# matthiasverstraete/3d_recognizer

Hardware: AMD Instinct MI355X
Metric: training clouds/sec, N=40960 pts, bs=8, at 1/2/4/8 GPUs; mIoU parity (higher is better)
Workload: dtype f32 storage/accumulate, bf16x3 MFMA in the wide GEMMs

## Files before the change

### 3d_recognizer_amd/csrc/pool.hip

```cpp
#include <string.h>

#include "rl_common.h"
#include <stdlib.h>

namespace {

#ifdef RL_POOL_PLAIN_STORES
#define RL_ST1 rl_stx
#define RL_ST4 rl_stx4
#else
#define RL_ST1 rl_stx_nt
#define RL_ST4 rl_stx4_nt
#endif

typedef float f32x4 __attribute__((ext_vector_type(4)));
typedef __attribute__((ext_vector_type(4))) __bf16 bf16x4;
typedef __attribute__((ext_vector_type(8))) __bf16 bf16x8;
typedef __attribute__((ext_vector_type(4))) short s16x4;

typedef float f32x2 __attribute__((ext_vector_type(2)));
typedef __attribute__((ext_vector_type(2))) __bf16 bf16x2;
__device__ __forceinline__ void split2(const f32x2 x, unsigned& hi, unsigned& lo) {
    const unsigned hb = __builtin_bit_cast(unsigned, __builtin_convertvector(x, bf16x2));
    const f32x2 hf = {__uint_as_float(hb << 16), __uint_as_float(hb & 0xffff0000u)};
// ... 569 lines not shown
#pragma unroll
                    for (int r = 0; r < 4; ++r) accw[nb][kb][r] += red[((nb * DT + kb) * 4 + r) * 64 + lane];
        }
    }
    if (wave == 0) {
        float* out = p.slab + (long)blockIdx.x * p.slab_stride;
#pragma unroll
        for (int nb = 0; nb < DT; ++nb)
#pragma unroll
            for (int kb = 0; kb < DT; ++kb)
#pragma unroll
                for (int r = 0; r < 4; ++r) out[(long)(nb * 16 + lj * 4 + r) * D + kb * 16 + li] = accw[nb][kb][r];
    }
}

template <bool GB, bool XO = true>
__global__ __launch_bounds__(512) void pool128_bwd_kernel(const PoolParams p) {
    __shared__ __attribute__((aligned(16))) float lfm[LFold<8>::LDS_FLOATS];
    constexpr int NW = 8;
    constexpr int TERMS = 3;
    constexpr int DT = 8, D = 128, H = 64, XS = Tile<DT>::XS, XSB = Tile<DT>::XSB;
    __shared__ __attribute__((aligned(16))) __bf16 Wh[D * XSB];
    __shared__ __attribute__((aligned(16))) __bf16 Wl[D * XSB];
    __shared__ __attribute__((aligned(16))) float Tiles[NW][16 * XS];
    const int lane = threadIdx.x & 63, wave = __builtin_amdgcn_readfirstlane(threadIdx.x >> 6);
    const int li = lane & 15, lj = lane >> 4;
    for (int e = threadIdx.x; e < D * D; e += 64 * NW) {
        const int o = e / D, i = e - o * D;
        const float w = p.W[e];
        const __bf16 h = (__bf16)w;
        Wh[o * XSB + i] = h;
        if constexpr (TERMS == 3) Wl[o * XSB + i] = (__bf16)(w - (float)h);
    }
    LFold<DT> lf;
    lf.init(p, lj, lfm);
    __syncthreads();
    float* Xs = Tiles[wave];
    float* Ds = Tiles[wave];

    const PointSpan span = point_span<NW>(p, wave);
    const long pstep = span.step, Pend = span.end;
    long pt = span.first;
    int idx_cur = pt < Pend ? p.idx[pt * 16 + li] : 0;
    int idx_nxt = pt + pstep < Pend ? p.idx[(pt + pstep) * 16 + li] : 0;
    float4 raw[DT];
    Cursor cu;
    cu.start(pt, p.n);
    float gp[DT], gp_nxt[DT];
#pragma unroll
    for (int nb = 0; nb < DT; ++nb) gp[nb] = gp_nxt[nb] = 0.f;
    if (pt < Pend) {
        fetch_x<DT>(p, cu, li, lj, idx_cur, raw);
#pragma unroll
        for (int nb = 0; nb < DT; ++nb) gp[nb] = p.dP[pt * D + nb * 16 + li];
    }
    loads_landed();
    for (; pt < Pend; pt += pstep) {
        const Cursor cn = cu.next(pstep, p.n);
        float4 xa[DT];
        finish_x<DT>(p, li, lj, raw, lf, xa, Xs);
        const int idx_n2 = pt + 2 * pstep < Pend ? p.idx[(pt + 2 * pstep) * 16 + li] : 0;
        const Cursor cf = pt + pstep < Pend ? cn : cu;
        fetch_x<DT>(p, cf, li, lj, pt + pstep < Pend ? idx_nxt : idx_cur, raw);
#pragma unroll
        for (int nb = 0; nb < DT; ++nb) gp_nxt[nb] = p.dP[cf.pt * D + nb * 16 + li];
        loads_issued();
        cu = cn;
        idx_cur = idx_nxt; idx_nxt = idx_n2;
        if constexpr (XO)
#pragma unroll
            for (int c = 0; c < DT; ++c) rl_stx4<GB>(p.X_out, (pt * 16 + li) * D + 16 * c + 4 * lj, xa[c]);
        f32x4 a[DT];
#pragma unroll
        for (int nb = 0; nb < DT; ++nb) a[nb] = (f32x4){0.f, 0.f, 0.f, 0.f};
        tile_gemm_bf<DT>(xa, Wh, Wl, li, lj, a);
// ... 54 lines not shown
        __builtin_amdgcn_wave_barrier();
        const long orow = (pt * 16 + li) * H;
        float4 gold[DT / 2];
        if (p.gu_accumulate) {
#pragma unroll
            for (int c = 0; c < DT / 2; ++c) gold[c] = *reinterpret_cast<const float4*>(p.GU + orow + 16 * c + 4 * lj);
        }
#pragma unroll
        for (int c = DT / 2; c < DT; ++c)
            rl_stx4<GB>(p.DG, orow + 16 * c + 4 * lj - H, *reinterpret_cast<const float4*>(Ds + li * XS + 16 * c + 4 * lj));
#pragma unroll
        for (int c = 0; c < DT / 2; ++c) {
            f32x4 v = *reinterpret_cast<const f32x4*>(Ds + li * XS + 16 * c + 4 * lj);
            if (p.gu_accumulate) v += v4(gold[c]);
            *reinterpret_cast<float4*>(p.GU + orow + 16 * c + 4 * lj) = f4(v);
        }
#pragma unroll
        for (int nb = 0; nb < DT; ++nb) gp[nb] = gp_nxt[nb];
        __builtin_amdgcn_wave_barrier();
    }
}

struct RpeBwdParams {
    PoolParams pp;
    const float* G;
    double* stats;
    const float* coef;
    float* slab;
    float* GU1;
    int g_bf16;
};

__device__ __forceinline__ float li_sum(float v) {
    v += __shfl_xor(v, 1, 64); v += __shfl_xor(v, 2, 64); v += __shfl_xor(v, 4, 64); v += __shfl_xor(v, 8, 64);
// ... 1419 lines not shown
#pragma unroll
        for (int j = 0; j < 16; ++j) t += red[j][ex];
        dW[e] = t;
    }
}

enum PoolEntry { PE_FWD, PE_BWD, PE_STATS, PE_BN_REDUCE, PE_WGRAD };

struct PoolFacts {
    PoolEntry entry;
    int d, stage;
    int terms;
    bool rows_bf16, gu_accumulate, fwd_stats2;
    long points;
    bool skip_x;
};

typedef void (*PoolFn)();
struct PoolPlan {
    PoolFn fn;
    int grid, threads;
    int xcd_chunk;
    int dw_count;
    const char* name;
    const char* refusal;
};

constexpr int pool_wavefronts(bool virtual_bwd, int d) { return d == 128 || (virtual_bwd && d == 64) ? 8 : 4; }

template <template <int, int> class Pick, class... A>
PoolFn by_width(int d, int terms, A... a) {
    if (terms == 0) return d == 16 ? Pick<1, 0>::fn(a...) : d == 32 ? Pick<2, 0>::fn(a...) : Pick<4, 0>::fn(a...);
    return d == 16 ? Pick<1, 3>::fn(a...) : d == 32 ? Pick<2, 3>::fn(a...) : Pick<4, 3>::fn(a...);
}
template <int DT, int T> struct PoolFwd { static PoolFn fn() { return (PoolFn)pool_fwd_kernel<DT, T>; } };
template <int DT, int T> struct PoolBwd {
    static PoolFn fn(bool gb) {
        if constexpr (T == 3) if (gb) return (PoolFn)pool_bwd_kernel<DT, 3, false, 4, true>;
        return (PoolFn)pool_bwd_kernel<DT, T>;
// ... 30 lines not shown
    pl.threads = 64 * nw;
    const long per = 4 * nw;
    const long cap = rpe ? RL_MAX_SLOTS : nw == 8 ? 256 : (fwd && d <= 16) ? 1280 : (fwd && d == 64) ? 768 : 1024;
    const long g = (f.points + per - 1) / per;
    pl.grid = (int)(g < 1 ? 1 : g < cap ? g : cap);
    if (((fwd && virt) || f.entry == PE_STATS) && pl.grid >= 8 && pl.grid % 8 == 0 && f.points < (1l << 30))
        pl.xcd_chunk = (int)((f.points + 7) / 8);

    if (!(d == 16 || d == 32 || d == 64 || (d == 128 && !virt && !rpe && f.terms != 0))) {
        pl.refusal = "d must be 16, 32 or 64, or 128 with a stored U outside the fp32 arithmetic mode";
        return pl;
    }
    const bool gb = f.rows_bf16 && !fwd && f.entry != PE_STATS;
    if (gb && f.terms != 3 && d != 128) { pl.refusal = "bf16 gradient rows need the bf16x3 arithmetic mode"; return pl; }
    if (f.skip_x && gb) { pl.refusal = "bf16 gradient rows need X_out (the in-place X of the weight gradient is fp32 only)"; return pl; }
    switch (f.entry) {
    case PE_FWD:
        pl.name = virt ? "vpool_fwd_kernel" : d == 16 ? "pool_fwd_kernel<1>" : d == 32 ? "pool_fwd_kernel<2>" : d == 64 ? "pool_fwd_kernel<4>" : "pool_fwd_kernel<8>";
        pl.fn = virt ? by_width<VPoolFwd>(d, f.terms, s2, f.fwd_stats2)
              : d == 128 ? (PoolFn)pool_fwd_kernel<8, 3, pool_wavefronts(false, 128)> : by_width<PoolFwd>(d, f.terms);
        break;
    case PE_BWD:
        pl.name = virt ? "vpool_bwd_kernel" : d == 16 ? "pool_bwd_kernel<1>" : d == 32 ? "pool_bwd_kernel<2>" : d == 64 ? "pool_bwd_kernel<4>" : "pool128_bwd_kernel";
        pl.fn = virt ? by_width<VPoolBwd>(d, f.terms, s2, gb, f.gu_accumulate)
              : d == 128 ? (gb ? (PoolFn)pool128_bwd_kernel<true> : f.skip_x ? (PoolFn)pool128_bwd_kernel<false, false> : (PoolFn)pool128_bwd_kernel<false>)
              : by_width<PoolBwd>(d, f.terms, gb);
        pl.dw_count = d == 128 ? 0 : d * d;
        break;
    case PE_STATS:
        pl.name = "vrpe_stats_kernel";
        pl.fn = by_width<RpeStats>(d, f.terms, s2);
        break;
    case PE_BN_REDUCE:
    case PE_WGRAD:
        pl.name = f.entry == PE_WGRAD ? "vrpe_wgrad_kernel" : "vrpe_bn_reduce_kernel";
        pl.fn = by_width<RpeBwd>(d, f.terms, s2, gb, f.entry == PE_WGRAD);
        break;
    }
    return pl;
}

template <class... Args>
int launch_pool(const PoolPlan& pl, const char* who, void* stream, const float* slab, float* dW, Args... args) {
    hipStream_t st = (hipStream_t)stream;
    void (*fn)(Args...) = (void (*)(Args...))pl.fn;
    hipLaunchKernelGGL(fn, dim3(pl.grid), dim3(pl.threads), 0, st, args...);
    rl_note_kernel(pl.name);
    RL_LAUNCH_CHECK(who);
    if (dW) {
        hipLaunchKernelGGL(pool_dw_reduce_kernel, dim3(rl_cdiv(pl.dw_count, 16)), dim3(256), 0, st, slab, pl.grid, pl.dw_count, dW);
        RL_LAUNCH_CHECK(who);
    }
    return RL_OK;
// ... 45 lines not shown
    if (rc) return rc;
    RL_REQUIRE(d->G && d->W && (p->src > 0 || d->U) && d->g_bstride >= d->n, RL_ERR_ARGS, "%s: null G / W / U, or g_bstride < n", who);
    RL_REQUIRE((p->src > 0 || ((uintptr_t)d->U & 15) == 0) && ((uintptr_t)d->G & 15) == 0, RL_ERR_ARGS, "%s: U/G must be 16-byte aligned", who);
    RL_REQUIRE((d->u_scale == nullptr) == (d->u_shift == nullptr) && (d->g_scale == nullptr) == (d->g_shift == nullptr),
               RL_ERR_ARGS, "%s: scale/shift must come together", who);
    p->U = d->U; p->ulazy.scale = d->u_scale; p->ulazy.shift = d->u_shift; p->ulazy.act = d->u_act; p->ulazy.slope = d->u_slope;
    p->G = d->G; p->g_bstride = d->g_bstride;
    p->glazy.scale = d->g_scale; p->glazy.shift = d->g_shift; p->glazy.act = d->g_act; p->glazy.slope = d->g_slope;
    p->W = d->W;
    p->Pout = d->Pout; p->dP = d->dP; p->GU = d->GU; p->gu_accumulate = d->gu_accumulate; p->DG = d->DG; p->slab = d->slab;
    p->slab_stride = (long)d->d * d->d + (d->dW ? 0 : d->d);
    if (backward) p->piv1 = p->piv2 = nullptr;
    p->fstats2 = backward ? nullptr : d->bn_fwd_stats2;
    RL_REQUIRE(!p->fstats2 || (p->src == 1 && d->W2 && d->b2), RL_ERR_ARGS, "%s: bn_fwd_stats2 needs virtual stage 1 and W2 / b2", who);
    p->bstats = backward ? d->bn_bwd_stats : nullptr;
    RL_REQUIRE(!p->bstats || p->src > 0, RL_ERR_ARGS, "%s: bn_bwd_stats needs a virtual rpe stage", who);
    RL_REQUIRE(backward ? (d->dP && d->GU && d->DG) : d->Pout != nullptr, RL_ERR_ARGS, "%s: null output / gradient buffers", who);
    return RL_OK;
}

int plan_grid(PoolEntry entry, int64_t points, int d, int stage) { return plan_pool({entry, d, stage, rl_wide_terms(), false, false, false, points}).grid; }

}

extern "C" int rl_pool_supported(int d, int nbr_k) { return nbr_k == 16 && !plan_pool({PE_FWD, d, 0, rl_wide_terms(), false, false, false, 1}).refusal; }

extern "C" int64_t rl_pool_slab_floats(int64_t points, int d) {
    const int stored = plan_grid(PE_BWD, points, d, 0), virt = plan_grid(PE_BWD, points, d, 1);
    return (int64_t)(stored > virt ? stored : virt) * (d * d + d);
}
extern "C" int rl_pool_bwd_slots(int64_t points, int d) { return plan_grid(PE_BWD, points, d, 1); }
// ... 3 lines not shown
extern "C" int64_t rl_rpe_wgrad_slab_floats(int64_t points, int d, int stage) {
    const int h = d / 2;
    return (int64_t)plan_grid(PE_WGRAD, points, d, stage) * ((int64_t)h * (stage == 1 ? 10 : h) + h);
}

extern "C" int rl_pool_fwd(const rl_pool_desc* d, void* stream) {
    PoolParams p;
    int rc = fill(&p, d, "rl_pool_fwd", false);
    if (rc) return rc;
    const PoolPlan pl = plan_pool({PE_FWD, p.d, p.src, rl_wide_terms(), false, false, p.fstats2 != nullptr, p.P});
    RL_REQUIRE(!pl.refusal, RL_ERR_UNSUPPORTED, "rl_pool_fwd: %s (d %d, u_source %d)", pl.refusal, p.d, p.src);
    p.xcd_chunk = pl.xcd_chunk;
    return launch_pool(pl, "rl_pool_fwd", stream, nullptr, nullptr, p);
}

extern "C" int rl_pool_bwd(const rl_pool_desc* d, void* stream) {
    PoolParams p;
    int rc = fill(&p, d, "rl_pool_bwd", true);
    if (rc) return rc;
    const bool skip_x = p.d == 128 && d->x_optional != 0 && d->X_out == nullptr;
    const PoolPlan pl = plan_pool({PE_BWD, p.d, p.src, rl_wide_terms(), d->rows_bf16 != 0, p.gu_accumulate != 0, false, p.P, skip_x});
    RL_REQUIRE(!pl.refusal, RL_ERR_UNSUPPORTED, "rl_pool_bwd: %s (d %d, u_source %d)", pl.refusal, p.d, p.src);
    if (p.d == 128) {
        RL_REQUIRE((d->X_out || skip_x) && d->dS_out, RL_ERR_ARGS, "rl_pool_bwd: d = 128 needs X_out and dS_out");
        RL_REQUIRE((((uintptr_t)d->X_out | (uintptr_t)d->dS_out) & 15) == 0, RL_ERR_ARGS, "rl_pool_bwd: X_out / dS_out must be 16-byte aligned");
        p.X_out = d->X_out; p.dS_out = d->dS_out;
        return launch_pool(pl, "rl_pool_bwd", stream, nullptr, nullptr, p);
    }
    RL_REQUIRE(d->slab, RL_ERR_ARGS, "rl_pool_bwd: null gradient buffers");
    RL_REQUIRE(d->slab_floats >= (int64_t)pl.grid * p.slab_stride, RL_ERR_ARGS, "rl_pool_bwd: slab too small");
    return launch_pool(pl, "rl_pool_bwd", stream, p.slab, d->dW, p);
}

static int g_pool128_x_in_place = 1;
extern "C" int rl_set_pool128_x(const char* mode) {
    const bool in_place = mode && !strcmp(mode, "in_place"), stored = mode && !strcmp(mode, "stored");
    RL_REQUIRE(in_place || stored, RL_ERR_ARGS, "rl_set_pool128_x: mode must be \"in_place\" or \"stored\"");
    g_pool128_x_in_place = in_place ? 1 : 0;
    return RL_OK;
}
extern "C" const char* rl_get_pool128_x(void) { return g_pool128_x_in_place ? "in_place" : "stored"; }

extern "C" int rl_rpe_stats(const rl_pool_desc* d, double* stats, void* stream) {
    PoolParams p;
    int rc = fill_branch(&p, d, "rl_rpe_stats", BN_BELOW);
    if (rc) return rc;
    RL_REQUIRE(p.src > 0 && stats, RL_ERR_ARGS, "rl_rpe_stats: needs u_source 1 or 2 and a stats buffer");
// ... 41 lines not shown
```

### 3d_recognizer_amd/randlanet/_engine.py

```python
from dataclasses import dataclass, field
from typing import ClassVar, Dict, List, Optional

import torch

from . import _hip as H
from . import _ops as ops
from ._ops import Lazy, Rpe

BN_EPS = 1e-6
BN_MOMENTUM = 0.99
BN_PIVOT = True
BAND_SORT_MIN_POINTS = 4096
POOL_X_IN_PLACE_MIN_ROWS = 2048
DECODER_CAT_IN_PLACE_MIN_ROWS = 8192


@dataclass(slots=True, eq=False)
class _Record:
    kind: ClassVar[str] = ""
    level: int = field(default=-1, init=False)


@dataclass(slots=True, eq=False)
class LinearRec(_Record):
    kind: ClassVar[str] = "linear"
    a: object
    out: Lazy
    wname: str
    bname: Optional[str]
# ... 17 lines not shown
    d: int


@dataclass(slots=True, eq=False)
class PoolFusedRec(_Record):
    kind: ClassVar[str] = "pool_fused"
    name: str
    u: object
    g: Lazy
    csr: object
    idx: torch.Tensor
    pooled: Lazy
    n: int
    d: int
    stage: int


@dataclass(slots=True, eq=False)
class AddActRec(_Record):
    kind: ClassVar[str] = "add_act"
    m2: Lazy
    sc: Lazy
    O: Lazy


@dataclass(slots=True, eq=False)
class InterpConcatRec(_Record):
    kind: ClassVar[str] = "interp_concat"
    prev: Lazy
    skip: Lazy
# ... 207 lines not shown
        for Y, (wname, bname, bn, n_out, act, slope, ks, ns, stats), last in zip(res, metas, (first_is_last_consumer, 0)):
            out = Lazy(Y, a.B, a.n, a.n, n_out)
            self._bn(ctx, out, stats, bn, act, slope, folded_bias=self.P[bname],
                     nslots=H.row_blocks(out.rows, 128) if stats is not None else None)
            ctx.record(LinearRec(a, out, wname, bname, ks, ns, True, last))
            outs.append(out)
        return outs[0], outs[1]

    def _mlp(self, ctx, a, name: str, n_out: int, act: int = H.ACT_NONE, slope: float = 0.0, *, transposed=False,
             bn=True, a_grad=True, last_consumer_of_input: int = 0) -> Lazy:
        return self._linear(ctx, a, f"{name}.conv.weight", f"{name}.conv.bias", n_out, transposed=transposed,
                            bn=f"{name}.batch_norm" if bn else None, act=act, slope=slope, a_grad=a_grad,
                            last_consumer_of_input=last_consumer_of_input)

    def _pool(self, ctx, name: str, u, g: Lazy, idx: torch.Tensor, csr, n: int, d: int, n_out: int, stage: int = 0,
              next_stats: bool = False) -> Lazy:
        B, K, h = u.B, self.K, d // 2
        rows = B * n * K
        Ws = self.P[f"{name}.score_fn.0.weight"]
        if ops.pool_supported(d, K):
            if next_stats:
                res, st2, ns2 = ops.pool_fwd(u, g, idx, Ws, n, d, stage, next_stats=True)
                ctx.next_stats = (st2, ns2)
            else:
                res = ops.pool_fwd(u, g, idx, Ws, n, d, stage)
            pooled = ops.plain(res, B, n)
            ctx.record(PoolFusedRec(name, u, g, csr, idx, pooled, n, d, stage))
            return self._mlp(ctx, pooled, f"{name}.mlp", n_out, H.ACT_RELU)
        X = self._pool_x_in_place(ctx, u, g, idx, Ws, n, d)
        if X is None:
            X = torch.empty((rows, d), dtype=torch.float32, device=u.raw.device)
            ops.copy_rows_pair(((u.raw, (0, h), n * K, X, (0, h), rows, n * K), dict(lazy=u)),
                               ((g.raw, (0, h), g.bstride, X, (h, h), rows, n * K), dict(index=idx, lazy=g)))
            S = ops.gemm(ops.plain(X, B, n * K), Ws, 1, d, d, None, wsplit=ctx.wsplit)
        else:
            S = ops.gemm(X, Ws, 1, d, d, None, wsplit=ctx.wsplit)
        Pt = ops.attpool_fwd(X, S, B * n, K)
        pooled = ops.plain(Pt, B, n)
        ctx.record(PoolRec(name, u, g, csr, X, S, pooled, n, d))
        return self._mlp(ctx, pooled, f"{name}.mlp", n_out, H.ACT_RELU)

    def _pool_x_in_place(self, ctx, u, g: Lazy, idx: torch.Tensor, Ws: torch.Tensor, n: int, d: int):
# ... 42 lines not shown
            vr.piv1, vr.piv2 = self._pivot(ctx, f"{e}.mlp_rpe1.batch_norm"), self._pivot(ctx, f"{e}.mlp_rpe2.batch_norm")
            vr.bn1 = self._virtual_bn(ctx, vr, 1, f"{e}.mlp_rpe1.batch_norm")
            ops.bn_finalize_flush(ctx.bn_defer)
            q1 = self._pool(ctx, f"{e}.pool1", vr, f0, idx, csr, n, d, h, stage=1, next_stats=ctx.training)
            vr.bn2 = self._virtual_bn(ctx, vr, 2, f"{e}.mlp_rpe2.batch_norm", *ctx.next_stats)
            ctx.next_stats = (None, 1)
            ops.bn_finalize_flush(ctx.bn_defer)
            ctx.bn_defer = None
            q2 = self._pool(ctx, f"{e}.pool2", vr, q1, idx, csr, n, d, d, stage=2)
        else:
            rpe = Rpe(xyz, idx, d2, B, n, K)
            if h <= 128:
                rpe = ops.rpe_build(rpe)
            u1 = self._mlp(ctx, rpe, f"{e}.mlp_rpe1", h, H.ACT_RELU, a_grad=False)
            ops.bn_finalize_flush(ctx.bn_defer)
            q1 = self._pool(ctx, f"{e}.pool1", u1, f0, idx, csr, n, d, h)
            u2 = self._mlp(ctx, u1, f"{e}.mlp_rpe2", h, H.ACT_RELU)
            ops.bn_finalize_flush(ctx.bn_defer)
            ctx.bn_defer = None
            q2 = self._pool(ctx, f"{e}.pool2", u2, q1, idx, csr, n, d, d)
        m2 = self._mlp(ctx, q2, f"{e}.mlp2", 2 * d, last_consumer_of_input=1)
        O = ops.plain(ops.add_act_fwd(m2, sc, 0.01), B, n)
        ctx.record(AddActRec(m2, sc, O))
        return O

    def _wide_weight_uses(self, training: bool):
        uses = []
        for name, W in self.P.items():
            if not name.endswith(("conv.weight", "score_fn.0.weight")) or W.dim() < 2:
                continue
            a, b = int(W.shape[0]), int(W.shape[1])
            if max(a, b) <= 64:
                if name.endswith(".mlp1.conv.weight") and b % 32 == 0 and b > 64:
                    sc = self.P.get(name.replace(".mlp1.", ".shortcut."))
                    if sc is not None and int(sc.shape[0]) > 64:
# ... 220 lines not shown
                assert ga.written == (r.last_consumer_of_input == 2), wname
            complete = (bool(r.last_consumer_of_input) and self.sync is None and a.scale is not None and a.mean is not None
                        and a.rows == a.raw.shape[0])
            res = ops.gemm(gl, self._w2(wname), ns, ks, a.C, None, out=ga.buf, out_bstride=a.bstride, accumulate=ga.written,
                           wsplit=st.wsplit, bnb=a if complete else None)
            if complete and res[1] is not None:
                st.bn_pre[id(a.raw)] = res[1]
            ga.written = True

    def _bwd_pool_fused(self, st: _Backward, r: PoolFusedRec):
        if r.stage:
            return self._bwd_pool_virtual(st, r)
        u, g, n, d = r.u, r.g, r.n, r.d
        GP = st.arrived(r.pooled).buf
        gu, gg = st.slot(u), st.slot(g)
        DG = ops.pool_bwd(u, g, r.idx, self.P[f"{r.name}.score_fn.0.weight"], n, d, GP, gu.buf, gu.written,
                          st.grads[f"{r.name}.score_fn.0.weight"], pending=st.pending, batch=st.wbatch)
        gu.written = True
        ops.segment_sum_rows(DG, (0, d // 2), n * self.K, r.csr, gg.buf, g.bstride, accumulate=gg.written)
        gg.written = True

    def _bwd_add_act(self, st: _Backward, r: AddActRec):
        m2, sc, O, grads = r.m2, r.sc, r.O, st.grads
        G = st.arrived(O).buf
        if ops.resid_bn_supported(m2, sc):
            g2 = ops.resid_bn_backward(G, O.raw, 0.01, m2, sc, grads[f"{m2.bn}.weight"], grads[f"{m2.bn}.bias"],
                                       grads[f"{sc.bn}.weight"], grads[f"{sc.bn}.bias"], sync=self.sync)
            st.bn_done.update((id(m2.raw), id(sc.raw)))
        else:
            ops.add_act_bwd(G, O.raw, 0.01)
            g2 = torch.empty_like(G)
            ops.copy_rows(G, (0, O.C), O.n, g2, (0, O.C), O.rows, O.n)
# ... 92 lines not shown
```

### 3d_recognizer_amd/randlanet/_hip.py

```python
import ctypes as C
import os
from typing import Optional

import torch

_LIB: Optional[C.CDLL] = None
_LIB_PATH = os.path.join(os.path.dirname(os.path.dirname(os.path.abspath(__file__))), "csrc",
                         "librandla_hip.so")
_LIB_PATH = os.environ.get("RL_HIP_LIB", _LIB_PATH)

ABI_VERSION = 110
MAX_SLOTS = 1024
KNN_MAX_K = 64
ACT_NONE, ACT_RELU, ACT_LRELU = 0, 1, 2

ERR_ARGS, ERR_FEW_SUPPORT, ERR_LAUNCH, ERR_UNSUPPORTED = -1, -2, -3, -4


class HipKernelError(RuntimeError):
    pass


class GemmDesc(C.Structure):
    _fields_ = [
# ... 113 lines not shown
        ("G", C.c_void_p), ("g_bstride", C.c_int64), ("g_scale", C.c_void_p), ("g_shift", C.c_void_p),
        ("g_act", C.c_int32), ("g_slope", C.c_float),
        ("idx", C.c_void_p), ("W", C.c_void_p), ("points", C.c_int64),
        ("n", C.c_int32), ("d", C.c_int32), ("nbr_k", C.c_int32),
        ("Pout", C.c_void_p), ("dP", C.c_void_p), ("GU", C.c_void_p), ("gu_accumulate", C.c_int32),
        ("DG", C.c_void_p), ("dW", C.c_void_p), ("slab", C.c_void_p), ("slab_floats", C.c_int64),
        ("X_out", C.c_void_p), ("dS_out", C.c_void_p),
        ("u_source", C.c_int32), ("xyz", C.c_void_p), ("xyz_bstride", C.c_int64), ("nbr_d2", C.c_void_p),
        ("W1", C.c_void_p), ("b1", C.c_void_p), ("scale1", C.c_void_p), ("shift1", C.c_void_p),
        ("W2", C.c_void_p), ("b2", C.c_void_p), ("scale2", C.c_void_p), ("shift2", C.c_void_p),
        ("mean1", C.c_void_p), ("invstd1", C.c_void_p), ("mean2", C.c_void_p), ("invstd2", C.c_void_p),
        ("xyz_width", C.c_int32), ("bn_bwd_stats", C.c_void_p), ("bn_fwd_stats2", C.c_void_p),
        ("rows_bf16", C.c_int32),
        ("pivot_mean1", C.c_void_p), ("pivot_mean2", C.c_void_p),
        ("x_optional", C.c_int32),
    ]


class ResidBnBwdDesc(C.Structure):
    _fields_ = [
        ("G", C.c_void_p), ("G2", C.c_void_p), ("O", C.c_void_p), ("slope", C.c_float), ("rows", C.c_int64), ("C", C.c_int32),
        ("Y1", C.c_void_p), ("scale1", C.c_void_p), ("mean1", C.c_void_p), ("invstd1", C.c_void_p),
        ("Y2", C.c_void_p), ("scale2", C.c_void_p), ("mean2", C.c_void_p), ("invstd2", C.c_void_p),
        ("stats1", C.c_void_p), ("stats2", C.c_void_p), ("coef1", C.c_void_p), ("coef2", C.c_void_p),
    ]


class CsrTask(C.Structure):
    _fields_ = [
        ("idx", C.c_void_p), ("n_src", C.c_int32), ("k", C.c_int32), ("n_dst", C.c_int32),
# ... 110 lines not shown
    "rl_segment_sum_rows": (_i, [C.POINTER(SegsumDesc), _vp]),
    "rl_pool_supported": (_i, [_i, _i]),
    "rl_pool_slab_floats": (_l, [_l, _i]),
    "rl_pool_bwd_slots": (_i, [_l, _i]),
    "rl_pool_bwd_grid": (_i, [_l, _i, _i]),
    "rl_pool_fwd_slots": (_i, [_l, _i]),
    "rl_pool_fwd": (_i, [C.POINTER(PoolDesc), _vp]),
    "rl_rpe_stats_slots": (_i, [_l]),
    "rl_rpe_stats": (_i, [C.POINTER(PoolDesc), _vp, _vp]),
    "rl_rpe_bn_reduce": (_i, [C.POINTER(PoolDesc), _vp, _vp, _vp]),
    "rl_rpe_wgrad_slab_floats": (_l, [_l, _i, _i]),
    "rl_rpe_wgrad": (_i, [C.POINTER(PoolDesc), _vp, _vp, _vp, _l, _vp, _vp]),
    "rl_pool_bwd": (_i, [C.POINTER(PoolDesc), _vp]),
    "rl_set_pool128_x": (_i, [C.c_char_p]),
    "rl_get_pool128_x": (C.c_char_p, []),
    "rl_set_pool256_x": (_i, [C.c_char_p]),
    "rl_get_pool256_x": (C.c_char_p, []),
    "rl_set_decoder_cat": (_i, [C.c_char_p]),
    "rl_get_decoder_cat": (C.c_char_p, []),
    "rl_gemm_concat_supported": (_i, [C.POINTER(GemmDesc)]),
    "rl_attpool_cat_supported": (_i, [C.POINTER(AttpoolSrc), _l, _i, _i]),
    "rl_attpool_fwd_cat": (_i, [C.POINTER(AttpoolSrc), _vp, _l, _i, _i, _vp, _vp]),
    "rl_attpool_bwd_cat": (_i, [C.POINTER(AttpoolSrc), _vp, _vp, _vp, _l, _i, _i, _vp, _vp, _vp]),
    "rl_attpool_fwd": (_i, [_vp, _vp, _l, _i, _i, _vp, _vp]),
    "rl_attpool_bwd": (_i, [_vp, _vp, _vp, _vp, _l, _i, _i, _vp, _vp, _vp]),
    "rl_add_act_fwd": (_i, [_vp, _vp, _vp, _vp, _vp, _vp, _l, _i, _f, _vp, _vp]),
    "rl_add_act_bwd": (_i, [_vp, _vp, _l, _i, _f, _vp]),
    "rl_rpe_build": (_i, [_vp, _l, _vp, _vp, _i, _i, _i, _vp, _vp]),
    "rl_rpe_build_dist": (_i, [_vp, _l, _vp, _vp, _i, _i, _i, _vp, _vp]),
    "rl_batch_assemble": (_i, [_vp, _i, _i, _i, _vp, _vp, _vp, _vp, _vp, _vp]),
# ... 126 lines not shown
            "tile": tuple(tile), "ksplit": ksplit.value, "reduce_cols": rcols.value}


def wgrad_plan(d: WgradDesc) -> dict:
    grid = (C.c_int32 * 3)()
    threads, nsplit, batch, rpb = C.c_int32(), C.c_int32(), C.c_int32(), C.c_int64()
    kernel, variant = C.c_char_p(), C.c_char_p()
    rc = lib().rl_wgrad_plan2(C.byref(d), grid, C.byref(threads), C.byref(kernel), C.byref(nsplit), C.byref(rpb), C.byref(batch),
                              C.byref(variant))
    if rc != 0:
        return {"rc": rc}
    return {"rc": 0, "kernel": kernel.value.decode(), "variant": variant.value.decode(), "grid": tuple(grid), "threads": threads.value,
            "nsplit": nsplit.value, "rows_per_block": rpb.value, "batch": batch.value}


_RAW_STREAM = getattr(torch._C, "_cuda_getCurrentRawStream", None)
_GET_DEVICE = getattr(torch._C, "_cuda_getDevice", None)


def stream_ptr(device=None) -> int:
    if _RAW_STREAM is not None and _GET_DEVICE is not None and device is None:
        return _RAW_STREAM(_GET_DEVICE())
    return torch.cuda.current_stream(device).cuda_stream


def current_device() -> int:
    return _GET_DEVICE() if _GET_DEVICE is not None else torch.cuda.current_device()


def ptr(t: Optional[torch.Tensor]) -> Optional[int]:
# ... 7 lines not shown
```

### 3d_recognizer_amd/randlanet/_ops.py

```python
import contextlib
import ctypes as C
import os
from dataclasses import dataclass
from typing import Optional, Tuple

import torch

from . import _hip as H

F32 = torch.float32
BF16 = torch.bfloat16

_STORAGE = os.environ.get("RL_STORAGE", "f32")


def set_storage(mode: str) -> None:
    global _STORAGE
    if mode not in ("f32", "bf16"):
        raise ValueError(f"storage must be 'f32' or 'bf16', got {mode!r}")
    if mode == "bf16" and get_wide_gemm() == "fp32":
        raise H.HipKernelError("bf16 storage needs the bf16x3 / bf16 arithmetic mode (RL_WIDE_GEMM)")
    _STORAGE = mode


# ... 281 lines not shown

    @property
    def rows(self) -> int:
        return self.skip.rows


_CONCAT = (ConcatGather, InterpConcat)


def set_pool128_x(mode: str) -> None:
    H.check(H.lib().rl_set_pool128_x(mode.encode()), "rl_set_pool128_x")


def get_pool128_x() -> str:
    return H.lib().rl_get_pool128_x().decode()


def set_pool256_x(mode: str) -> None:
    H.check(H.lib().rl_set_pool256_x(mode.encode()), "rl_set_pool256_x")


def get_pool256_x() -> str:
    return H.lib().rl_get_pool256_x().decode()


def set_decoder_cat(mode: str) -> None:
    H.check(H.lib().rl_set_decoder_cat(mode.encode()), "rl_set_decoder_cat")


def get_decoder_cat() -> str:
# ... 752 lines not shown
        pd.bn_fwd_stats2 = stats2.data_ptr()
    out = torch.empty((u.B * n, d), dtype=F32, device=W.device)
    pd.Pout = out.data_ptr()
    P = u.B * n
    virt = isinstance(u, VirtualRpe)
    fbytes = P * (4 * (32 + d) + 16 * (16 + 4 * (d // 2))) if virt else 4 * (2 * P * 16 * (d // 2) + P * 16 + P * d)
    with _rec("pool_fwd_virtual" if virt else "pool_fwd", (P, 16, d), fbytes, 2 * P * 16 * d * d):
        H.check(H.lib().rl_pool_fwd(C.byref(pd), _st()), "rl_pool_fwd")
    if next_stats:
        return out, stats2, ns
    return out


def pool_bwd(u, g: Lazy, idx: torch.Tensor, W: torch.Tensor, n: int, d: int, dP: torch.Tensor,
             GU: torch.Tensor, gu_accumulate: bool, dW: torch.Tensor, pending: Optional[list] = None,
             stage: int = 0, bn_bwd_stats: Optional[torch.Tensor] = None, batch: Optional[list] = None) -> torch.Tensor:
    pd = _pool_desc(u, g, idx, W, n, d, stage)
    _dev_check(dP, GU, dW)
    P = u.B * n
    assert dP.shape == (P, d) and GU.shape == (P * 16, d // 2) and dW.numel() == d * d
    rdt = row_dtype()
    virt = isinstance(u, VirtualRpe)
    assert GU.dtype == (rdt if virt else F32), "GU: the row storage type under a virtual rpe branch, fp32 for a real U tensor"
    pd.rows_bf16 = int(rdt == BF16)
    es = 2 if rdt == BF16 else 4
    DG = torch.empty((P * 16, d // 2), dtype=rdt, device=W.device)
    if bn_bwd_stats is not None:
        _dev_check(bn_bwd_stats)
        assert stage > 0 and bn_bwd_stats.dtype == torch.float64
        assert bn_bwd_stats.numel() >= H.lib().rl_pool_bwd_slots(P, d) * d
        pd.bn_bwd_stats = bn_bwd_stats.data_ptr()
# ... 2 lines not shown
    if virt:
        nbytes = P * (4 * (32 + d) + 16 * (16 + 4 * h) + 4 * d + es * 16 * h * (2 + int(gu_accumulate)))
    else:
        nbytes = (4 * (2 * P * 16 * h + P * 16 + 2 * P * d) + es * P * 16 * h + 4 * P * 16 * h * (1 + int(gu_accumulate)))
    if d == 128:
        dS = torch.empty((P * 16, d), dtype=rdt, device=W.device)
        xop = ConcatGather(u, g, idx) if (rdt == F32 and not virt and get_pool128_x() == "in_place") else None
        if xop is not None and not wgrad_supported(xop, dS, n * 16, d):
            xop = None
        if xop is None:
            X = torch.empty((P * 16, d), dtype=rdt, device=W.device)
            pd.X_out, xop = X.data_ptr(), plain(X, u.B, n * 16)
        else:
            pd.x_optional = 1
        pd.dS_out = dS.data_ptr()
        with _rec("pool_bwd", (P, 16, d), nbytes + (1 + int(pd.x_optional == 0)) * es * P * 16 * d, 4 * P * 16 * d * d):
            H.check(H.lib().rl_pool_bwd(C.byref(pd), _st()), "rl_pool_bwd")
        wgrad(xop, dS, n * 16, d, dW, 1, d, None, pending=pending, batch=batch)
        return DG
    floats = H.lib().rl_pool_slab_floats(P, d)
    if pending is not None:
        slab = torch.empty(floats, dtype=F32, device=W.device)
        pd.dW = None
    else:
        slab = _slab(W.device, floats)
    pd.slab, pd.slab_floats = slab.data_ptr(), slab.numel()
    with _rec("pool_bwd", (P, 16, d), nbytes, 6 * P * 16 * d * d):
        H.check(H.lib().rl_pool_bwd(C.byref(pd), _st()), "rl_pool_bwd")
    if pending is not None:
        it = H.WgradReduceItem()
        it.slab, it.dW, it.dbias, it.w_ks, it.w_ns = slab.data_ptr(), dW.data_ptr(), None, 1, d
        it.nsplit, it.N, it.K = H.lib().rl_pool_bwd_grid(P, d, int(virt)), d, d
        pending.append((it, slab, dW, None))
    return DG


def _attpool_src(x: ConcatGather) -> H.AttpoolSrc:
    u, g, idx = x.u, x.g, x.idx
    _dev_check(u.raw, u.scale, u.shift, g.raw, g.scale, g.shift, idx)
    assert idx.dtype == torch.int32 and idx.numel() == u.rows and u.bstride == u.n and g.B == u.B and u.C == g.C
    assert u.raw.dtype == F32 and g.raw.dtype == F32 and u.raw.shape[0] >= u.rows and u.raw.shape[1] >= u.C
    assert g.raw.shape[0] >= (g.B - 1) * g.bstride + g.n and g.raw.shape[1] >= g.C, "second source rows out of range"
    d = H.AttpoolSrc()
    d.U, d.ldu, d.G, d.ldg, d.g_bstride = u.raw.data_ptr(), u.raw.shape[1], g.raw.data_ptr(), g.raw.shape[1], g.bstride
    if u.scale is not None:
        d.u_scale, d.u_shift, d.u_act, d.u_slope = u.scale.data_ptr(), u.shift.data_ptr(), u.act, u.slope
    if g.scale is not None:
        d.g_scale, d.g_shift, d.g_act, d.g_slope = g.scale.data_ptr(), g.shift.data_ptr(), g.act, g.slope
    assert u.n % 16 == 0
# ... 1002 lines not shown
```

### include/rl_randlanet.h

```cpp
#ifndef RL_RANDLANET_H
#define RL_RANDLANET_H

#include <stdint.h>

#ifdef __cplusplus
extern "C" {
#endif

#define RL_VERSION 110

#define RL_OK 0
#define RL_ERR_ARGS (-1)
#define RL_ERR_FEW_SUPPORT (-2)
#define RL_ERR_LAUNCH (-3)
#define RL_ERR_UNSUPPORTED (-4)

#define RL_MAX_SLOTS 1024
#define RL_KNN_MAX_K 64
#define RL_MAX_CLASSES 256

const char* rl_last_error(void);
const char* rl_last_kernel(void);
int rl_version(void);
int64_t rl_launch_count(void);
// ... 352 lines not shown
    const float* W2;
    const float* b2;
    const float* scale2;
    const float* shift2;
    const float* mean1;
    const float* invstd1;
    const float* mean2;
    const float* invstd2;
    int32_t xyz_width;
    double* bn_bwd_stats;
    double* bn_fwd_stats2;
    int32_t rows_bf16;
    const float* pivot_mean1;
    const float* pivot_mean2;
    int32_t x_optional;
} rl_pool_desc;

int rl_pool_supported(int d, int nbr_k);
int64_t rl_pool_slab_floats(int64_t points, int d);
int rl_pool_bwd_slots(int64_t points, int d);
int rl_pool_bwd_grid(int64_t points, int d, int virtual_stage);
int rl_pool_fwd_slots(int64_t points, int d);
int rl_pool_fwd(const rl_pool_desc* d, void* stream);
int rl_pool_bwd(const rl_pool_desc* d, void* stream);
int rl_set_pool128_x(const char* mode);
const char* rl_get_pool128_x(void);

int rl_rpe_stats_slots(int64_t points);
int rl_rpe_stats(const rl_pool_desc* d, double* stats, void* stream);

int rl_rpe_bn_reduce(const rl_pool_desc* d, const float* G, double* stats, void* stream);
int64_t rl_rpe_wgrad_slab_floats(int64_t points, int d, int stage);
int rl_rpe_wgrad(const rl_pool_desc* d, const float* G, const float* coef, float* slab, int64_t slab_floats,
                 float* GU1, void* stream);

int rl_add_act_fwd(const float* Y1, const float* s1, const float* b1, const float* Y2,
                   const float* s2, const float* b2, int64_t rows, int C, float slope, float* O,
                   void* stream);
int rl_add_act_bwd(float* G, const float* O, int64_t rows, int C, float slope, void* stream);

int rl_rpe_build(const float* xyz, int64_t xyz_bstride, const int32_t* nbr_idx, const float* nbr_d2, int B,
// ... 242 lines not shown
```

Baseline: 1312.

## Fuse BatchNorm-backward sums into the d=128 pool backward kernel

Adds a variant of pool128_bwd_kernel that, while writing the GU gradient rows, also accumulates the per-channel BatchNorm-backward sums (sum of gated gradient and gradient times normalized input) for the stored U, and reduces them per block into a double slab. The engine requests it when this pool is the last consumer of U and the rows exceed a threshold, and hands the partial sums to the BN backward stage. This is meant to save a separate sweep over the large GU/U tensors. It adds registers, LDS and a block-level reduction inside a hot kernel, which may lower occupancy, and the engine-side use of st.bn_pre is not shown.

```diff
diff --git a/3d_recognizer_amd/csrc/pool.hip b/3d_recognizer_amd/csrc/pool.hip
--- a/3d_recognizer_amd/csrc/pool.hip
+++ b/3d_recognizer_amd/csrc/pool.hip
@@ -607,9 +607,11 @@
     }
 }
 
-template <bool GB, bool XO = true>
+__device__ __forceinline__ float li_sum(float v);
+template <bool GB, bool XO = true, bool BS = false>
 __global__ __launch_bounds__(512) void pool128_bwd_kernel(const PoolParams p) {
-    __shared__ __attribute__((aligned(16))) float lfm[LFold<8>::LDS_FLOATS];
+    static_assert(!(BS && GB), "the BatchNorm-backward sums are left by the fp32-row kernel only");
+    __shared__ __attribute__((aligned(16))) float lfm[LFold<8>::LDS_FLOATS + (BS ? 2 * 64 : 0)];
     constexpr int NW = 8;
     constexpr int TERMS = 3;
     constexpr int DT = 8, D = 128, H = 64, XS = Tile<DT>::XS, XSB = Tile<DT>::XSB;
@@ -627,6 +629,14 @@
     }
     LFold<DT> lf;
     lf.init(p, lj, lfm);
+    const float* bnm = lfm + LFold<DT>::LDS_FLOATS + 4 * lj;
+    if constexpr (BS)
+        if (threadIdx.x < 2 * H) lfm[LFold<DT>::LDS_FLOATS + threadIdx.x] = threadIdx.x < H ? p.mu1[threadIdx.x] : p.is1[threadIdx.x - H];
+    const float neg = eff_slope(p.ulazy);
+    f32x4 bsg[BS ? DT / 2 : 1], bsx[BS ? DT / 2 : 1];
+    if constexpr (BS)
+#pragma unroll
+        for (int c = 0; c < DT / 2; ++c) bsg[c] = bsx[c] = splat(0.f);
     __syncthreads();
     float* Xs = Tiles[wave];
     float* Ds = Tiles[wave];
@@ -652,6 +662,10 @@
         const Cursor cn = cu.next(pstep, p.n);
         float4 xa[DT];
         finish_x<DT>(p, li, lj, raw, lf, xa, Xs);
+        float4 yu[BS ? DT / 2 : 1];
+        if constexpr (BS)
+#pragma unroll
+            for (int c = 0; c < DT / 2; ++c) yu[c] = raw[c];
         const int idx_n2 = pt + 2 * pstep < Pend ? p.idx[(pt + 2 * pstep) * 16 + li] : 0;
         const Cursor cf = pt + pstep < Pend ? cn : cu;
         fetch_x<DT>(p, cf, li, lj, pt + pstep < Pend ? idx_nxt : idx_cur, raw);
@@ -736,10 +750,44 @@
             f32x4 v = *reinterpret_cast<const f32x4*>(Ds + li * XS + 16 * c + 4 * lj);
             if (p.gu_accumulate) v += v4(gold[c]);
             *reinterpret_cast<float4*>(p.GU + orow + 16 * c + 4 * lj) = f4(v);
+            if constexpr (BS) {
+                const f32x4 y = v4(yu[c]), z = y * lf.sc(c) + lf.sh(c);
+                f32x4 g;
+#pragma unroll
+                for (int r = 0; r < 4; ++r) g[r] = v[r] * (z[r] > 0.f ? 1.f : neg);
+                const f32x4 xh = (y - *reinterpret_cast<const f32x4*>(bnm + 16 * c)) * *reinterpret_cast<const f32x4*>(bnm + H + 16 * c);
+                bsg[c] += g;
+                bsx[c] = __builtin_elementwise_fma(g, xh, bsx[c]);
+            }
         }
 #pragma unroll
         for (int nb = 0; nb < DT; ++nb) gp[nb] = gp_nxt[nb];
         __builtin_amdgcn_wave_barrier();
+    }
+    if constexpr (BS) {
+        __syncthreads();
+        double* redd = reinterpret_cast<double*>(&Tiles[0][0]);
+#pragma unroll
+        for (int c = 0; c < DT / 2; ++c)
+#pragma unroll
+            for (int r = 0; r < 4; ++r) {
+                const float sa = li_sum(bsg[c][r]), sb = li_sum(bsx[c][r]);
+                if (li == 0) {
+                    redd[(wave * 2 + 0) * H + 16 * c + 4 * lj + r] = (double)sa;
+                    redd[(wave * 2 + 1) * H + 16 * c + 4 * lj + r] = (double)sb;
+                }
+            }
+        __syncthreads();
+        if (threadIdx.x < H) {
+            const int c = threadIdx.x;
+            double a0 = 0.0, a1 = 0.0;
+            for (int wv = 0; wv < NW; ++wv) {
+                a0 += redd[(wv * 2 + 0) * H + c];
+                a1 += redd[(wv * 2 + 1) * H + c];
+            }
+            p.bstats[((long)blockIdx.x * 2 + 0) * H + c] = a0;
+            p.bstats[((long)blockIdx.x * 2 + 1) * H + c] = a1;
+        }
     }
 }
 
@@ -2189,6 +2237,7 @@
     bool rows_bf16, gu_accumulate, fwd_stats2;
     long points;
     bool skip_x;
+    bool bn_sums;
 };
 
 typedef void (*PoolFn)();
@@ -2198,6 +2247,7 @@
     int xcd_chunk;
     int dw_count;
     const char* name;
+    const char* variant;
     const char* refusal;
 };
 
@@ -2258,6 +2308,9 @@
     const bool gb = f.rows_bf16 && !fwd && f.entry != PE_STATS;
     if (gb && f.terms != 3 && d != 128) { pl.refusal = "bf16 gradient rows need the bf16x3 arithmetic mode"; return pl; }
     if (f.skip_x && gb) { pl.refusal = "bf16 gradient rows need X_out (the in-place X of the weight gradient is fp32 only)"; return pl; }
+    const bool bs = f.bn_sums && f.entry == PE_BWD && !virt;
+    if (bs && d != 128) { pl.refusal = "bn_bwd_stats with a stored U needs d = 128"; return pl; }
+    if (bs && gb) { pl.refusal = "bn_bwd_stats with a stored U needs fp32 gradient rows"; return pl; }
     switch (f.entry) {
     case PE_FWD:
         pl.name = virt ? "vpool_fwd_kernel" : d == 16 ? "pool_fwd_kernel<1>" : d == 32 ? "pool_fwd_kernel<2>" : d == 64 ? "pool_fwd_kernel<4>" : "pool_fwd_kernel<8>";
@@ -2267,9 +2320,13 @@
     case PE_BWD:
         pl.name = virt ? "vpool_bwd_kernel" : d == 16 ? "pool_bwd_kernel<1>" : d == 32 ? "pool_bwd_kernel<2>" : d == 64 ? "pool_bwd_kernel<4>" : "pool128_bwd_kernel";
         pl.fn = virt ? by_width<VPoolBwd>(d, f.terms, s2, gb, f.gu_accumulate)
+              : bs ? (f.skip_x ? (PoolFn)pool128_bwd_kernel<false, false, true> : (PoolFn)pool128_bwd_kernel<false, true, true>)
               : d == 128 ? (gb ? (PoolFn)pool128_bwd_kernel<true> : f.skip_x ? (PoolFn)pool128_bwd_kernel<false, false> : (PoolFn)pool128_bwd_kernel<false>)
               : by_width<PoolBwd>(d, f.terms, gb);
         pl.dw_count = d == 128 ? 0 : d * d;
+        if (d == 128 && !virt)
+            pl.variant = bs ? (f.skip_x ? "pool128_bwd_kernel<fp32,no_x,bn_sums>" : "pool128_bwd_kernel<fp32,x,bn_sums>")
+                       : gb ? "pool128_bwd_kernel<bf16,x>" : f.skip_x ? "pool128_bwd_kernel<fp32,no_x>" : "pool128_bwd_kernel<fp32,x>";
         break;
     case PE_STATS:
         pl.name = "vrpe_stats_kernel";
@@ -2281,6 +2338,7 @@
         pl.fn = by_width<RpeBwd>(d, f.terms, s2, gb, f.entry == PE_WGRAD);
         break;
     }
+    if (!pl.variant) pl.variant = pl.name;
     return pl;
 }
 
@@ -2356,7 +2414,11 @@
     p->fstats2 = backward ? nullptr : d->bn_fwd_stats2;
     RL_REQUIRE(!p->fstats2 || (p->src == 1 && d->W2 && d->b2), RL_ERR_ARGS, "%s: bn_fwd_stats2 needs virtual stage 1 and W2 / b2", who);
     p->bstats = backward ? d->bn_bwd_stats : nullptr;
-    RL_REQUIRE(!p->bstats || p->src > 0, RL_ERR_ARGS, "%s: bn_bwd_stats needs a virtual rpe stage", who);
+    RL_REQUIRE(!p->bstats || p->src > 0 || d->d == 128, RL_ERR_ARGS, "%s: bn_bwd_stats needs a virtual rpe stage, or d = 128", who);
+    if (p->bstats && p->src == 0) {
+        RL_REQUIRE(d->u_scale && d->u_mean && d->u_invstd, RL_ERR_ARGS, "%s: bn_bwd_stats with a stored U needs u_scale / u_shift and u_mean / u_invstd", who);
+        p->mu1 = d->u_mean; p->is1 = d->u_invstd;
+    }
     RL_REQUIRE(backward ? (d->dP && d->GU && d->DG) : d->Pout != nullptr, RL_ERR_ARGS, "%s: null output / gradient buffers", who);
     return RL_OK;
 }
@@ -2390,23 +2452,54 @@
     return launch_pool(pl, "rl_pool_fwd", stream, nullptr, nullptr, p);
 }
 
-extern "C" int rl_pool_bwd(const rl_pool_desc* d, void* stream) {
-    PoolParams p;
+static int pool_bwd_plan(const rl_pool_desc* d, PoolParams* pp, PoolPlan* plan) {
+    PoolParams& p = *pp;
     int rc = fill(&p, d, "rl_pool_bwd", true);
     if (rc) return rc;
     const bool skip_x = p.d == 128 && d->x_optional != 0 && d->X_out == nullptr;
-    const PoolPlan pl = plan_pool({PE_BWD, p.d, p.src, rl_wide_terms(), d->rows_bf16 != 0, p.gu_accumulate != 0, false, p.P, skip_x});
+    const PoolPlan pl = *plan = plan_pool({PE_BWD, p.d, p.src, rl_wide_terms(), d->rows_bf16 != 0, p.gu_accumulate != 0, false, p.P, skip_x,
+                                           p.bstats != nullptr && p.src == 0});
     RL_REQUIRE(!pl.refusal, RL_ERR_UNSUPPORTED, "rl_pool_bwd: %s (d %d, u_source %d)", pl.refusal, p.d, p.src);
     if (p.d == 128) {
         RL_REQUIRE((d->X_out || skip_x) && d->dS_out, RL_ERR_ARGS, "rl_pool_bwd: d = 128 needs X_out and dS_out");
         RL_REQUIRE((((uintptr_t)d->X_out | (uintptr_t)d->dS_out) & 15) == 0, RL_ERR_ARGS, "rl_pool_bwd: X_out / dS_out must be 16-byte aligned");
         p.X_out = d->X_out; p.dS_out = d->dS_out;
-        return launch_pool(pl, "rl_pool_bwd", stream, nullptr, nullptr, p);
+        return RL_OK;
     }
     RL_REQUIRE(d->slab, RL_ERR_ARGS, "rl_pool_bwd: null gradient buffers");
     RL_REQUIRE(d->slab_floats >= (int64_t)pl.grid * p.slab_stride, RL_ERR_ARGS, "rl_pool_bwd: slab too small");
+    return RL_OK;
+}
+
+extern "C" int rl_pool_bwd(const rl_pool_desc* d, void* stream) {
+    PoolParams p;
+    PoolPlan pl;
+    int rc = pool_bwd_plan(d, &p, &pl);
+    if (rc) return rc;
+    if (p.d == 128) return launch_pool(pl, "rl_pool_bwd", stream, nullptr, nullptr, p);
     return launch_pool(pl, "rl_pool_bwd", stream, p.slab, d->dW, p);
 }
+
+extern "C" int rl_pool_bwd_plan(const rl_pool_desc* d, int32_t* grid, int32_t* threads, const char** kernel, const char** variant) {
+    PoolParams p;
+    PoolPlan pl;
+    int rc = pool_bwd_plan(d, &p, &pl);
+    if (rc) return rc;
+    if (grid) *grid = pl.grid;
+    if (threads) *threads = pl.threads;
+    if (kernel) *kernel = pl.name;
+    if (variant) *variant = pl.variant;
+    return RL_OK;
+}
+
+static int g_pool128_bn_sums_kernel = 1;
+extern "C" int rl_set_pool128_bn_sums(const char* mode) {
+    const bool kernel = mode && !strcmp(mode, "kernel"), sweep = mode && !strcmp(mode, "sweep");
+    RL_REQUIRE(kernel || sweep, RL_ERR_ARGS, "rl_set_pool128_bn_sums: mode must be \"kernel\" or \"sweep\"");
+    g_pool128_bn_sums_kernel = kernel ? 1 : 0;
+    return RL_OK;
+}
+extern "C" const char* rl_get_pool128_bn_sums(void) { return g_pool128_bn_sums_kernel ? "kernel" : "sweep"; }
 
 static int g_pool128_x_in_place = 1;
 extern "C" int rl_set_pool128_x(const char* mode) {
diff --git a/3d_recognizer_amd/randlanet/_engine.py b/3d_recognizer_amd/randlanet/_engine.py
--- a/3d_recognizer_amd/randlanet/_engine.py
+++ b/3d_recognizer_amd/randlanet/_engine.py
@@ -13,6 +13,8 @@
 BAND_SORT_MIN_POINTS = 4096
 POOL_X_IN_PLACE_MIN_ROWS = 2048
 DECODER_CAT_IN_PLACE_MIN_ROWS = 8192
+
+POOL128_BN_SUMS_MIN_ROWS = 8192
 
 
 @dataclass(slots=True, eq=False)
@@ -60,6 +62,7 @@
     n: int
     d: int
     stage: int
+    last_consumer_of_u: int = 0
 
 
 @dataclass(slots=True, eq=False)
@@ -297,7 +300,7 @@
                             last_consumer_of_input=last_consumer_of_input)
 
     def _pool(self, ctx, name: str, u, g: Lazy, idx: torch.Tensor, csr, n: int, d: int, n_out: int, stage: int = 0,
-              next_stats: bool = False) -> Lazy:
+              next_stats: bool = False, last_consumer_of_u: int = 0) -> Lazy:
         B, K, h = u.B, self.K, d // 2
         rows = B * n * K
         Ws = self.P[f"{name}.score_fn.0.weight"]
@@ -308,7 +311,7 @@
             else:
                 res = ops.pool_fwd(u, g, idx, Ws, n, d, stage)
             pooled = ops.plain(res, B, n)
-            ctx.record(PoolFusedRec(name, u, g, csr, idx, pooled, n, d, stage))
+            ctx.record(PoolFusedRec(name, u, g, csr, idx, pooled, n, d, stage, last_consumer_of_u))
             return self._mlp(ctx, pooled, f"{name}.mlp", n_out, H.ACT_RELU)
         X = self._pool_x_in_place(ctx, u, g, idx, Ws, n, d)
         if X is None:
@@ -381,11 +384,11 @@
                 rpe = ops.rpe_build(rpe)
             u1 = self._mlp(ctx, rpe, f"{e}.mlp_rpe1", h, H.ACT_RELU, a_grad=False)
             ops.bn_finalize_flush(ctx.bn_defer)
-            q1 = self._pool(ctx, f"{e}.pool1", u1, f0, idx, csr, n, d, h)
+            q1 = self._pool(ctx, f"{e}.pool1", u1, f0, idx, csr, n, d, h, last_consumer_of_u=2)
             u2 = self._mlp(ctx, u1, f"{e}.mlp_rpe2", h, H.ACT_RELU)
             ops.bn_finalize_flush(ctx.bn_defer)
             ctx.bn_defer = None
-            q2 = self._pool(ctx, f"{e}.pool2", u2, q1, idx, csr, n, d, d)
+            q2 = self._pool(ctx, f"{e}.pool2", u2, q1, idx, csr, n, d, d, last_consumer_of_u=1)
         m2 = self._mlp(ctx, q2, f"{e}.mlp2", 2 * d, last_consumer_of_input=1)
         O = ops.plain(ops.add_act_fwd(m2, sc, 0.01), B, n)
         ctx.record(AddActRec(m2, sc, O))
@@ -636,8 +639,15 @@
         u, g, n, d = r.u, r.g, r.n, r.d
         GP = st.arrived(r.pooled).buf
         gu, gg = st.slot(u), st.slot(g)
-        DG = ops.pool_bwd(u, g, r.idx, self.P[f"{r.name}.score_fn.0.weight"], n, d, GP, gu.buf, gu.written,
-                          st.grads[f"{r.name}.score_fn.0.weight"], pending=st.pending, batch=st.wbatch)
+        if r.last_consumer_of_u:
+            assert gu.written == (r.last_consumer_of_u == 2), r.name
+        want = (bool(r.last_consumer_of_u) and d == 128 and self.sync is None and u.rows > POOL128_BN_SUMS_MIN_ROWS
+                and u.scale is not None and u.mean is not None and ops.get_pool128_bn_sums() == "kernel")
+        res = ops.pool_bwd(u, g, r.idx, self.P[f"{r.name}.score_fn.0.weight"], n, d, GP, gu.buf, gu.written,
+                           st.grads[f"{r.name}.score_fn.0.weight"], pending=st.pending, batch=st.wbatch, want_bn_sums=want)
+        DG, pre = res if want else (res, None)
+        if pre is not None:
+            st.bn_pre[id(u.raw)] = pre
         gu.written = True
         ops.segment_sum_rows(DG, (0, d // 2), n * self.K, r.csr, gg.buf, g.bstride, accumulate=gg.written)
         gg.written = True
diff --git a/3d_recognizer_amd/randlanet/_hip.py b/3d_recognizer_amd/randlanet/_hip.py
--- a/3d_recognizer_amd/randlanet/_hip.py
+++ b/3d_recognizer_amd/randlanet/_hip.py
@@ -151,6 +151,7 @@
         ("rows_bf16", C.c_int32),
         ("pivot_mean1", C.c_void_p), ("pivot_mean2", C.c_void_p),
         ("x_optional", C.c_int32),
+        ("u_mean", C.c_void_p), ("u_invstd", C.c_void_p),
     ]
 
 
@@ -291,6 +292,9 @@
     "rl_pool_bwd": (_i, [C.POINTER(PoolDesc), _vp]),
     "rl_set_pool128_x": (_i, [C.c_char_p]),
     "rl_get_pool128_x": (C.c_char_p, []),
+    "rl_pool_bwd_plan": (_i, [C.POINTER(PoolDesc), C.POINTER(C.c_int32), C.POINTER(C.c_int32), C.POINTER(C.c_char_p), C.POINTER(C.c_char_p)]),
+    "rl_set_pool128_bn_sums": (_i, [C.c_char_p]),
+    "rl_get_pool128_bn_sums": (C.c_char_p, []),
     "rl_set_pool256_x": (_i, [C.c_char_p]),
     "rl_get_pool256_x": (C.c_char_p, []),
     "rl_set_decoder_cat": (_i, [C.c_char_p]),
@@ -447,6 +451,15 @@
             "nsplit": nsplit.value, "rows_per_block": rpb.value, "batch": batch.value}
 
 
+def pool_bwd_plan(d: PoolDesc) -> dict:
+    grid, threads = C.c_int32(), C.c_int32()
+    kernel, variant = C.c_char_p(), C.c_char_p()
+    rc = lib().rl_pool_bwd_plan(C.byref(d), C.byref(grid), C.byref(threads), C.byref(kernel), C.byref(variant))
+    if rc != 0:
+        return {"rc": rc}
+    return {"rc": 0, "kernel": kernel.value.decode(), "variant": variant.value.decode(), "grid": grid.value, "threads": threads.value}
+
+
 _RAW_STREAM = getattr(torch._C, "_cuda_getCurrentRawStream", None)
 _GET_DEVICE = getattr(torch._C, "_cuda_getDevice", None)
 
diff --git a/3d_recognizer_amd/randlanet/_ops.py b/3d_recognizer_amd/randlanet/_ops.py
--- a/3d_recognizer_amd/randlanet/_ops.py
+++ b/3d_recognizer_amd/randlanet/_ops.py
@@ -319,6 +319,14 @@
 
 def get_pool128_x() -> str:
     return H.lib().rl_get_pool128_x().decode()
+
+
+def set_pool128_bn_sums(mode: str) -> None:
+    H.check(H.lib().rl_set_pool128_bn_sums(mode.encode()), "rl_set_pool128_bn_sums")
+
+
+def get_pool128_bn_sums() -> str:
+    return H.lib().rl_get_pool128_bn_sums().decode()
 
 
 def set_pool256_x(mode: str) -> None:
@@ -1101,7 +1109,8 @@
 
 def pool_bwd(u, g: Lazy, idx: torch.Tensor, W: torch.Tensor, n: int, d: int, dP: torch.Tensor,
              GU: torch.Tensor, gu_accumulate: bool, dW: torch.Tensor, pending: Optional[list] = None,
-             stage: int = 0, bn_bwd_stats: Optional[torch.Tensor] = None, batch: Optional[list] = None) -> torch.Tensor:
+             stage: int = 0, bn_bwd_stats: Optional[torch.Tensor] = None, batch: Optional[list] = None,
+             want_bn_sums: bool = False):
     pd = _pool_desc(u, g, idx, W, n, d, stage)
     _dev_check(dP, GU, dW)
     P = u.B * n
@@ -1134,10 +1143,22 @@
         else:
             pd.x_optional = 1
         pd.dS_out = dS.data_ptr()
+        pre = None
+        if want_bn_sums and not virt and rdt == F32 and u.scale is not None and u.mean is not None:
+            _dev_check(u.mean, u.invstd)
+            nslots = H.lib().rl_pool_bwd_grid(P, d, 0)
+            sums = torch.empty((nslots, 2, h), dtype=torch.float64, device=W.device)
+            pd.bn_bwd_stats, pd.u_mean, pd.u_invstd = sums.data_ptr(), u.mean.data_ptr(), u.invstd.data_ptr()
+            rc = H.lib().rl_pool_bwd_plan(C.byref(pd), None, None, None, None)
+            if rc == H.ERR_UNSUPPORTED:
+                pd.bn_bwd_stats = pd.u_mean = pd.u_invstd = None
+            else:
+                H.check(rc, "rl_pool_bwd_plan")
+                pre = (sums, nslots)
         with _rec("pool_bwd", (P, 16, d), nbytes + (1 + int(pd.x_optional == 0)) * es * P * 16 * d, 4 * P * 16 * d * d):
             H.check(H.lib().rl_pool_bwd(C.byref(pd), _st()), "rl_pool_bwd")
         wgrad(xop, dS, n * 16, d, dW, 1, d, None, pending=pending, batch=batch)
-        return DG
+        return (DG, pre) if want_bn_sums else DG
     floats = H.lib().rl_pool_slab_floats(P, d)
     if pending is not None:
         slab = torch.empty(floats, dtype=F32, device=W.device)
@@ -1152,7 +1173,7 @@
         it.slab, it.dW, it.dbias, it.w_ks, it.w_ns = slab.data_ptr(), dW.data_ptr(), None, 1, d
         it.nsplit, it.N, it.K = H.lib().rl_pool_bwd_grid(P, d, int(virt)), d, d
         pending.append((it, slab, dW, None))
-    return DG
+    return (DG, None) if want_bn_sums else DG
 
 
 def _attpool_src(x: ConcatGather) -> H.AttpoolSrc:
diff --git a/include/rl_randlanet.h b/include/rl_randlanet.h
--- a/include/rl_randlanet.h
+++ b/include/rl_randlanet.h
@@ -390,6 +390,8 @@
     const float* pivot_mean1;
     const float* pivot_mean2;
     int32_t x_optional;
+    const float* u_mean;
+    const float* u_invstd;
 } rl_pool_desc;
 
 int rl_pool_supported(int d, int nbr_k);
@@ -401,6 +403,9 @@
 int rl_pool_bwd(const rl_pool_desc* d, void* stream);
 int rl_set_pool128_x(const char* mode);
 const char* rl_get_pool128_x(void);
+int rl_pool_bwd_plan(const rl_pool_desc* d, int32_t* grid, int32_t* threads, const char** kernel, const char** variant);
+int rl_set_pool128_bn_sums(const char* mode);
+const char* rl_get_pool128_bn_sums(void);
 
 int rl_rpe_stats_slots(int64_t points);
 int rl_rpe_stats(const rl_pool_desc* d, double* stats, void* stream);
```

Result: no change. 1325, median of 6 (+1.0%).
